# pr0g/ToyMeshPathTracer

Hardware: NVIDIA B200
Metric: Mrays/s (primary+bounce+shadow) (higher is better)
Workload: dtype f32

## Files before the change

toymeshpathtracer_b200/csrc/build_logic.cuh:

```cuda
#pragma once
#include "bvh.cuh"

namespace bld {

struct Box {
    float lox, loy, loz, hix, hiy, hiz;
};
TMPT_HD Box box_union(const Box& a, const Box& b) {
    return Box{fminf(a.lox, b.lox), fminf(a.loy, b.loy), fminf(a.loz, b.loz),
               fmaxf(a.hix, b.hix), fmaxf(a.hiy, b.hiy), fmaxf(a.hiz, b.hiz)};
}
TMPT_HD float box_half_area(const Box& b) {
    float dx = b.hix - b.lox, dy = b.hiy - b.loy, dz = b.hiz - b.loz;
    return dx * dy + dy * dz + dz * dx;
}

TMPT_HD uint32_t float_to_ordered(float f) {
    uint32_t u = ex::f2u(f);
    return (u & 0x80000000u) ? ~u : (u | 0x80000000u);
}
TMPT_HD float ordered_to_float(uint32_t u) {
    return ex::u2f((u & 0x80000000u) ? (u & 0x7FFFFFFFu) : ~u);
}

// ... 282 lines not shown
            const uint32_t wi = wideBase + (uint32_t)inner;
            refs[j] = wi;
            if (w.parent) w.parent[wi] = it.wide;
            outQueue[qBase + inner] = WorkItem{c[j], wi, it.depth + 1};
            ++inner;
        }
    }
    counter_max(&w.counters[3], (uint32_t)it.depth);
    float4* o = w.nodes + (size_t)it.wide * bvh::NODE_F4;
    o[0] = make_float4(lox[0], lox[1], lox[2], lox[3]);
    o[1] = make_float4(hix[0], hix[1], hix[2], hix[3]);
    o[2] = make_float4(loy[0], loy[1], loy[2], loy[3]);
    o[3] = make_float4(hiy[0], hiy[1], hiy[2], hiy[3]);
    o[4] = make_float4(loz[0], loz[1], loz[2], loz[3]);
    o[5] = make_float4(hiz[0], hiz[1], hiz[2], hiz[3]);
    o[6] = make_float4(ex::u2f(refs[0]), ex::u2f(refs[1]), ex::u2f(refs[2]), ex::u2f(refs[3]));
}

TMPT_HD void emit_single_leaf_root(const BinTree& t, const WideOut& w, int rootNode) {
    const int cnt = subtree_count(t, rootNode);
    const uint32_t first = counter_add(&w.counters[1], (uint32_t)cnt);
    counter_add(&w.counters[2], 1u);
    emit_leaf_tris(t, w, rootNode, first);
    const float4 lo = t.lo[rootNode], hi = t.hi[rootNode];
    const float F = 3.0e38f;
    float4* o = w.nodes;
    o[0] = make_float4(lo.x, F, F, F); o[1] = make_float4(hi.x, -F, -F, -F);
    o[2] = make_float4(lo.y, F, F, F); o[3] = make_float4(hi.y, -F, -F, -F);
    o[4] = make_float4(lo.z, F, F, F); o[5] = make_float4(hi.z, -F, -F, -F);
    o[6] = make_float4(ex::u2f(bvh::make_leaf_ref(first, cnt)), ex::u2f(bvh::NONE), ex::u2f(bvh::NONE), ex::u2f(bvh::NONE));
    accum_add(&w.sahAccum[1], box_half_area(Box{lo.x, lo.y, lo.z, hi.x, hi.y, hi.z}) * (float)cnt);
}


template <class LoadRow>
TMPT_HD void refit_wide_node(float4* nodes, float4* tris, const float* tris9, uint32_t node, float sceneMaxAbs, LoadRow ldnode) {
    float4* o = nodes + (size_t)node * bvh::NODE_F4;
    const float4 rf = o[6];
    const uint32_t refs[4] = {ex::f2u(rf.x), ex::f2u(rf.y), ex::f2u(rf.z), ex::f2u(rf.w)};
    float lo[3][4], hi[3][4];
    for (int k = 0; k < 4; ++k) {
        Box b{3.0e38f, 3.0e38f, 3.0e38f, -3.0e38f, -3.0e38f, -3.0e38f};
        if (refs[k] != bvh::NONE && bvh::ref_is_leaf(refs[k])) {
            const uint32_t first = bvh::leaf_first(refs[k]);
            for (int j = 0; j < bvh::leaf_count(refs[k]); ++j) {
                float4* slot = tris + (size_t)(first + j) * 3;
                const uint32_t id = ex::f2u(slot[0].w);
                const float* p = tris9 + (size_t)id * 9;
                const ex::V3 v0 = ex::v3(p[0], p[1], p[2]), v1 = ex::v3(p[3], p[4], p[5]), v2 = ex::v3(p[6], p[7], p[8]);
                const ex::V3 e1 = ex::sub(v1, v0), e2 = ex::sub(v2, v0);
                slot[0] = make_float4(v0.x, v0.y, v0.z, ex::u2f(id));
                slot[1] = make_float4(e1.x, e1.y, e1.z, 0.0f);
                slot[2] = make_float4(e2.x, e2.y, e2.z, 0.0f);
                Box tb = tri_box(p);
                const float dx = tb.hix - tb.lox, dy = tb.hiy - tb.loy, dz = tb.hiz - tb.loz;
                const float pad = pad_for(sqrtf(dx * dx + dy * dy + dz * dz), sceneMaxAbs);
                tb.lox -= pad; tb.loy -= pad; tb.loz -= pad; tb.hix += pad; tb.hiy += pad; tb.hiz += pad;
                b = box_union(b, tb);
            }
        } else if (refs[k] != bvh::NONE) {
            const float4 r0 = ldnode(refs[k], 0), r1 = ldnode(refs[k], 1), r2 = ldnode(refs[k], 2), r3 = ldnode(refs[k], 3), r4 = ldnode(refs[k], 4),
                         r5 = ldnode(refs[k], 5);
            b.lox = fminf(fminf(r0.x, r0.y), fminf(r0.z, r0.w)); b.hix = fmaxf(fmaxf(r1.x, r1.y), fmaxf(r1.z, r1.w));
            b.loy = fminf(fminf(r2.x, r2.y), fminf(r2.z, r2.w)); b.hiy = fmaxf(fmaxf(r3.x, r3.y), fmaxf(r3.z, r3.w));
            b.loz = fminf(fminf(r4.x, r4.y), fminf(r4.z, r4.w)); b.hiz = fmaxf(fmaxf(r5.x, r5.y), fmaxf(r5.z, r5.w));
        }
// ... 84 lines not shown
```

toymeshpathtracer_b200/csrc/bvh.cuh:

```cuda
#pragma once
#include "exact.cuh"
#include "sungrid.cuh"


#ifdef __CUDA_ARCH__
#define TMPT_LDG4(p) __ldg(p)
#else
#define TMPT_LDG4(p) (*(p))
#endif

namespace bvh {

constexpr uint32_t LEAF_BIT = 0x80000000u;
constexpr int MAX_LEAF_TRIS = 8;
constexpr int WIDTH = 4;
constexpr int NODE_F4 = 7;
constexpr int QNODE_ROWS = 4;
#ifndef TMPT_STACK_SIZE
#define TMPT_STACK_SIZE 128
#endif
constexpr int STACK_SIZE = TMPT_STACK_SIZE;
constexpr int MAX_TREE_DEPTH = (STACK_SIZE - 4) / 3;
constexpr uint32_t NONE = 0xFFFFFFFFu;
constexpr uint32_t STACK_OVERFLOW = 1;

TMPT_HD uint32_t make_leaf_ref(uint32_t firstSlot, int count) { return LEAF_BIT | (uint32_t(count - 1) << 28) | firstSlot; }
TMPT_HD bool ref_is_leaf(uint32_t r) { return (r & LEAF_BIT) != 0; }
TMPT_HD int leaf_count(uint32_t r) { return int((r >> 28) & 7u) + 1; }
TMPT_HD uint32_t leaf_first(uint32_t r) { return r & 0x0FFFFFFFu; }

struct SceneView {
    const float4* nodes;
    const float4* tris;
    const float* tris9;
    const float4* hitdata;
    uint32_t rootRef;
    int triCount;
    uint32_t* status;
    const uint4* qnodes;
    float farLimit;
    sun::View sun;
};

struct HitRec {
    int id;
    float t;
    float u, v;
};



TMPT_HD bool mt_exact(ex::V3 o, ex::V3 d, ex::V3 v0, ex::V3 e1, ex::V3 e2, float tMin, float tMax,
                      float& t, float& u, float& v) {
    const float Epsilon = 1e-5f;
    ex::V3 pvec = ex::cross(d, e2);
    float det = ex::dot(e1, pvec);
    float invDet = ex::rcp(det);
    ex::V3 tvec = ex::sub(o, v0);
    u = ex::mul(ex::dot(tvec, pvec), invDet);
    if ((det > -Epsilon && det < Epsilon) || u < 0.0f || u > 1.0f) return false;
    ex::V3 qvec = ex::cross(tvec, e1);
    v = ex::mul(ex::dot(d, qvec), invDet);
    if (v < 0.0f || ex::add(u, v) > 1.0f) return false;
    t = ex::mul(ex::dot(e2, qvec), invDet);
    return t >= tMin && t <= tMax;
}

TMPT_HD ex::V3 tri_normal(ex::V3 v0, ex::V3 v1, ex::V3 v2) { return ex::normalize(ex::cross(ex::sub(v1, v0), ex::sub(v2, v0))); }
TMPT_HD float4 ld_row_payload(const float4* p);
TMPT_HD void hit_payload(const SceneView& sc, int id, float u, float v, ex::V3& pos, ex::V3& normal) {
    ex::V3 v0, v1, v2;
    if (sc.hitdata) {
        const float4* h = sc.hitdata + (size_t)id * 3;
        const float4 a = ld_row_payload(h), b = ld_row_payload(h + 1), c = ld_row_payload(h + 2);
        v0 = ex::v3(a.x, a.y, a.z); v1 = ex::v3(b.x, b.y, b.z); v2 = ex::v3(c.x, c.y, c.z);
        normal = ex::v3(a.w, b.w, c.w);
    } else {
        const float* p = sc.tris9 + (size_t)id * 9;
        v0 = ex::v3(p[0], p[1], p[2]); v1 = ex::v3(p[3], p[4], p[5]); v2 = ex::v3(p[6], p[7], p[8]);
        normal = tri_normal(v0, v1, v2);
    }
    float w = ex::sub(ex::sub(1.0f, u), v);
    pos = ex::add(ex::add(ex::muls(v0, w), ex::muls(v1, u)), ex::muls(v2, v));
}

TMPT_HD float safe_dir(float d) { return fabsf(d) < 1.0e-20f ? copysignf(1.0e-20f, d) : d; }

struct TravStats {
    unsigned long long nodes = 0;
    unsigned long long tris = 0;
    unsigned long long iters = 0;
    unsigned long long culledPops = 0;
    unsigned long long leafWaits = 0;
    unsigned long long nodeWarps = 0;
    unsigned long long triWarps = 0;
    unsigned long long warpIters = 0;
    unsigned long long overflows = 0;
    unsigned long long depthOver[5] = {0, 0, 0, 0, 0};
    int maxSp = 0;
};

struct LocalStack {
    static constexpr bool kCanOverflow = false;
    unsigned long long e[STACK_SIZE];
    TMPT_HD bool put_if(bool push, int i, unsigned long long v) {
        if (push) e[i] = v;
        return push;
    }
    TMPT_HD unsigned long long get(int i) const { return *(const volatile unsigned long long*)&e[i]; }
    TMPT_HD bool overflowed() const { return false; }
    TMPT_HD void reset() {}
};
template <int S, int STRIDE>
struct SmemStack {
    static constexpr bool kCanOverflow = true;
    uint32_t col;
    bool ovf;
#ifdef __CUDA_ARCH__
    static __device__ __forceinline__ SmemStack make(const void* smemBase, uint32_t thread) {
        uint32_t a = (uint32_t)__cvta_generic_to_shared(smemBase) + thread * 8u, held;
        asm volatile("mov.u32 %0, %1;" : "=r"(held) : "r"(a));
        return SmemStack{held, false};
    }
    __device__ __forceinline__ bool put_if(bool push, int i, unsigned long long v) {
        const bool ok = push && i < S;
        if (ok) asm volatile("st.shared.u64 [%0], %1;" ::"r"(col + (uint32_t)i * (uint32_t)(STRIDE * 8)), "l"(v) : "memory");
        ovf = ovf || (push && !ok);
        return ok;
    }
    __device__ __forceinline__ unsigned long long get(int i) const {
        unsigned long long v;
// ... 313 lines not shown
#endif
    if (e == end) return false;
#ifdef __CUDA_ARCH__
    uint2 cur = __ldg(g.entries + e);
#else
    uint2 cur = g.entries[e];
#endif
    for (;;) {
        if (ex::u2f(cur.y) < w) return false;
        ++e;
        uint2 nxt = cur;
        if (e < end) {
#ifdef __CUDA_ARCH__
            nxt = __ldg(g.entries + e);
#else
            nxt = g.entries[e];
#endif
        }
        if (STATS) ++stats->tris;
        const uint32_t row0 = cur.x * 3u;
        const float4 a = ld_row_tri(sc.tris + row0), b = ld_row_tri(sc.tris + (row0 + 1u)), cc = ld_row_tri(sc.tris + (row0 + 2u));
        float t, bu, bv;
        if (mt_exact(p, l, ex::v3(a.x, a.y, a.z), ex::v3(b.x, b.y, b.z), ex::v3(cc.x, cc.y, cc.z), tMin, tMax, t, bu, bv)) return true;
        if (e >= end) return false;
        cur = nxt;
    }
}

struct WalkState {
    RayCtx r;
    ex::V3 o, d;
    HitRec best;
    uint32_t cur, triPos, triEnd;
    int sp;
    bool any;
};
TMPT_HD void walk_start(WalkState& w, const SceneView& sc, ex::V3 o, ex::V3 d, float tMax, bool any) {
    w.r = make_ray_ctx(o, d);
    w.o = o; w.d = d;
    w.best.id = -1; w.best.t = tMax; w.best.u = 0.0f; w.best.v = 0.0f;
    w.cur = ray_has_nan(o, d) ? NONE : sc.rootRef;
    w.triPos = 0; w.triEnd = 0;
    w.sp = 0;
    w.any = any;
}

TMPT_HD bool stats_any(bool pred) {
#ifdef __CUDA_ARCH__
    return __any_sync(__activemask(), pred);
#else
    return pred;
#endif
}
TMPT_HD bool stats_leader() {
#ifdef __CUDA_ARCH__
    const unsigned m = __activemask();
    unsigned lane;
    asm("mov.u32 %0, %%laneid;" : "=r"(lane));
    return (unsigned)(__ffs((int)m) - 1) == lane;
#else
    return true;
#endif
}

template <bool STATS, class Stack>
TMPT_HD bool walk_step(WalkState& w, const SceneView& sc, float tMin, float tMax, Stack& stack, TravStats* stats) {
    if (STATS) {
        ++stats->iters;
        const bool nodeAny = stats_any(w.cur != NONE && !ref_is_leaf(w.cur));
        if (stats_leader()) { ++stats->warpIters; stats->nodeWarps += nodeAny ? 1 : 0; }
    }
    if (w.cur != NONE && !ref_is_leaf(w.cur)) {
        if (STATS) ++stats->nodes;
        w.cur = node_step(sc, w.cur, w.r, tMin, w.best.t, stack, w.sp, w.any);
        if (STATS && w.sp > stats->maxSp) stats->maxSp = w.sp;
    }
    if (w.cur != NONE && ref_is_leaf(w.cur) && w.triPos == w.triEnd) {
        w.triPos = leaf_first(w.cur);
        w.triEnd = w.triPos + (uint32_t)leaf_count(w.cur);
        w.cur = NONE;
    }
    if (STATS) {
        if (w.cur != NONE && ref_is_leaf(w.cur)) ++stats->leafWaits;
        const bool triAny = stats_any(w.triPos < w.triEnd);
        if (stats_leader()) stats->triWarps += triAny ? 1 : 0;
    }
    const bool popping = w.cur == NONE && w.sp > 0;
    unsigned long long top = 0;
    if (popping) top = stack.get(w.sp - 1);
    if (w.triPos < w.triEnd) {
        if (STATS) ++stats->tris;
        if (tri_step(sc, w.triPos++, w.o, w.d, tMin, tMax, w.best) && w.any) return true;
    }
    if (popping) {
        --w.sp;
        if (ex::u2f((uint32_t)(top >> 32) & ~3u) <= w.best.t) w.cur = (uint32_t)top;
        else if (STATS) ++stats->culledPops;
    }
    const bool done = w.cur == NONE && w.triPos == w.triEnd && w.sp == 0;
    if (STATS && done) {
        const int lim[5] = {4, 8, 12, 16, 24};
        for (int k = 0; k < 5; ++k) stats->depthOver[k] += stats->maxSp > lim[k] ? 1 : 0;
        stats->maxSp = 0;
    }
    return done;
}

#ifdef __CUDA_ARCH__
// ... 12 lines not shown
            const int id = (int)ex::f2u(a.w);
            if (t < best.t || (t == best.t && best.id >= 0 && id < best.id)) { best.t = t; best.id = id; best.u = u; best.v = v; }
        }
    }
    return best;
}
TMPT_HD HitRec brute_force(const SceneView& sc, ex::V3 o, ex::V3 d, float tMin, float tMax) { return scan_all(sc.tris, sc.triCount, o, d, tMin, tMax); }

template <bool STATS>
TMPT_HD bool sun_query(const SceneView& sc, ex::V3 o, float tMin, float tMax, TravStats* stats) {
    const ex::V3 l = ex::v3(sc.sun.lx, sc.sun.ly, sc.sun.lz);
    if (ray_is_far(sc, o)) return scan_all(sc.tris, sc.triCount, o, l, tMin, tMax).id >= 0;
    return sun_occluded<STATS>(sc, o, l, tMin, tMax, stats);
}

template <bool ANY, bool STATS = false>
TMPT_HD HitRec traverse(const SceneView& sc, ex::V3 o, ex::V3 d, float tMin, float tMax, TravStats* stats = nullptr) {
    if (ray_is_far(sc, o)) return scan_all(sc.tris, sc.triCount, o, d, tMin, tMax);
    LocalStack stack;
    WalkState w;
    walk_start(w, sc, o, d, tMax, ANY);
    while (!walk_step<STATS>(w, sc, tMin, tMax, stack, stats)) {}
    return w.best;
}
template <bool ANY>
#ifdef __CUDA_ARCH__
__device__ __noinline__
#else
inline
#endif
HitRec traverse_again(const SceneView& sc, ex::V3 o, ex::V3 d, float tMin, float tMax) { return traverse<ANY, false>(sc, o, d, tMin, tMax); }

template <bool ANY, bool STATS, bool FAR, class Stack>
TMPT_HD HitRec traverse_with(Stack& stack, const SceneView& sc, ex::V3 o, ex::V3 d, float tMin, float tMax, TravStats* stats = nullptr) {
    if (FAR && ray_is_far(sc, o)) return scan_all(sc.tris, sc.triCount, o, d, tMin, tMax);
    WalkState w;
    walk_start(w, sc, o, d, tMax, ANY);
    while (!walk_step<STATS>(w, sc, tMin, tMax, stack, stats)) {}
    if (Stack::kCanOverflow && stack.overflowed()) {
        stack.reset();
        if (STATS) ++stats->overflows;
        if (!(ANY && w.best.id >= 0)) return traverse_again<ANY>(sc, o, d, tMin, tMax);
    }
    return w.best;
}

}
```

toymeshpathtracer_b200/csrc/integrator.cuh:

```cuda
#pragma once
#include "bvh.cuh"

namespace integ {

constexpr int kMaxDepth = 10;
constexpr float kMinT = 0.001f;
constexpr float kMaxT = 1.0e7f;

struct Camera {
    ex::V3 origin, lowerLeftCorner, horizontal, vertical, u, v, w;
    float lensRadius;
};

TMPT_HD void camera_get_ray(const Camera& c, float s, float t, uint32_t& rng, ex::V3& o, ex::V3& d) {
    float px, py;
    ex::random_in_unit_disk(rng, px, py);
    const float rdx = ex::mul(c.lensRadius, px), rdy = ex::mul(c.lensRadius, py);
    const ex::V3 offset = ex::add(ex::muls(c.u, rdx), ex::muls(c.v, rdy));
    o = ex::add(c.origin, offset);
    d = ex::normalize(ex::sub(ex::sub(ex::add(ex::add(c.lowerLeftCorner, ex::muls(c.horizontal, s)), ex::muls(c.vertical, t)), c.origin), offset));
}

TMPT_HD void primary_ray(const Camera& c, int x, int y, float invW, float invH, uint32_t& rng, ex::V3& o, ex::V3& d) {
    const float fv = ex::mul(ex::add((float)y, ex::random_float01(rng)), invH);
    const float fu = ex::mul(ex::add((float)x, ex::random_float01(rng)), invW);
    camera_get_ray(c, fu, fv, rng, o, d);
}

TMPT_HD ex::V3 sky(ex::V3 dir) {
    const float t = ex::mul(0.5f, ex::add(dir.y, 1.0f));
    const float a = ex::sub(1.0f, t);
    return ex::muls(ex::add(ex::v3(ex::mul(1.0f, a), ex::mul(1.0f, a), ex::mul(1.0f, a)), ex::muls(ex::v3(0.5f, 0.7f, 1.0f), t)), 0.5f);
}

TMPT_HD float sun_term(ex::V3 normal, ex::V3 rayDir, ex::V3 lightDir) {
    const ex::V3 nl = ex::dot(normal, rayDir) < 0.0f ? normal : ex::neg(normal);
    return fmaxf(0.0f, ex::dot(lightDir, nl));
}

// ... 2 lines not shown
    return ex::normalize(ex::sub(target, pos));
}

TMPT_HD ex::V3 unwind_step(float k, ex::V3 color) {
    const ex::V3 albedo = ex::v3(0.7f, 0.7f, 0.7f);
    const ex::V3 kLightColor = ex::v3(0.7f, 0.6f, 0.5f);
    const ex::V3 light = ex::add(ex::v3(0.0f, 0.0f, 0.0f), ex::muls(ex::mulv(albedo, kLightColor), k));
    return ex::add(light, ex::mulv(albedo, color));
}

TMPT_HD uchar4 resolve_pixel(ex::V3 sum, float sppRecip) {
    const ex::V3 c = ex::muls(sum, sppRecip);
    uchar4 px;
    px.x = ex::quantise(ex::sqrt_rn(c.x));
    px.y = ex::quantise(ex::sqrt_rn(c.y));
    px.z = ex::quantise(ex::sqrt_rn(c.z));
    px.w = 255;
    return px;
}

struct FirstHit {
    int id;
    float t;
    ex::V3 normal;
};

template <bool STATS = false, bool FAR = true, bool AOV = false, class Stack, class Scene>
TMPT_HD ex::V3 trace_path(Stack& stack, const Scene& sc, const Camera& cam, ex::V3 o, ex::V3 d, ex::V3 lightDir, uint32_t& rng,
                          unsigned long long& rays, bvh::TravStats* stats = nullptr, FirstHit* first = nullptr) {
    float kk[kMaxDepth];
    int depth = 0;
    ex::V3 color = ex::v3(0.0f, 0.0f, 0.0f);
    if (AOV) first->id = -1;
    while (depth < kMaxDepth) {
        ++rays;
        const bvh::HitRec h = bvh::traverse_with<false, STATS, FAR>(stack, sc, o, d, kMinT, kMaxT, stats);
        if (h.id < 0) { color = sky(d); break; }
        ex::V3 pos, normal;
        bvh::hit_payload(sc, h.id, h.u, h.v, pos, normal);
        if (AOV && depth == 0) { first->id = h.id; first->t = h.t; first->normal = normal; }
        ++rays;
#if defined(TMPT_SUN_ONLY) && TMPT_SUN_ONLY
        const bool shadowed = bvh::sun_occluded<STATS>(sc, pos, lightDir, kMinT, kMaxT, stats);
#else
        const bool shadowed = sc.sun.n > 0 ? bvh::sun_occluded<STATS>(sc, pos, lightDir, kMinT, kMaxT, stats)
                                           : bvh::traverse_with<true, STATS, FAR>(stack, sc, pos, lightDir, kMinT, kMaxT, stats).id >= 0;
#endif
        kk[depth] = shadowed ? 0.0f : sun_term(normal, d, lightDir);
        d = scatter_dir(pos, normal, rng);
        o = pos;
        ++depth;
    }
    for (int i = depth - 1; i >= 0; --i) color = unwind_step(kk[i], color);
    return color;
}

constexpr int kMaxChunkSamples = 8;
TMPT_HD int chunk_len(int spp) {
    const int c = spp / 32;
    return c < 1 ? 1 : c > kMaxChunkSamples ? kMaxChunkSamples : c;
}
TMPT_HD int chunk_count(int spp) { const int c = chunk_len(spp); return (spp + c - 1) / c; }

struct AovSums {
    ex::V3 normal;
    float t, hits;
    int id0;
};
TMPT_HD void aov_clear(AovSums& a) { a.normal = ex::v3(0.0f, 0.0f, 0.0f); a.t = 0.0f; a.hits = 0.0f; a.id0 = -1; }
TMPT_HD void aov_add_hit(AovSums& a, ex::V3 normal, float t) { a.normal = ex::add(a.normal, normal); a.t = ex::add(a.t, t); a.hits = ex::add(a.hits, 1.0f); }

TMPT_HD float4 radiance_of(ex::V3 sum, float sppRecip) {
    const ex::V3 c = ex::muls(sum, sppRecip);
    return make_float4(c.x, c.y, c.z, 1.0f);
}
TMPT_HD float4 normal_of(ex::V3 normalSum, float hits, float sppRecip) {
    const ex::V3 n = ex::muls(normalSum, sppRecip);
    return make_float4(n.x, n.y, n.z, ex::mul(hits, sppRecip));
}
// ... 58 lines not shown
```

toymeshpathtracer_b200/csrc/kernels.cu:

```cuda
#include <cooperative_groups.h>
#include <cuda_runtime.h>

#include <atomic>
#include <chrono>
#include <cmath>
#include <cstdarg>
#include <cstdio>
#include <cstdlib>
#include <cstring>
#include <mutex>
#include <new>
#include <string>
#include <vector>

#include "build_logic.cuh"
#include "common.h"
#include "denoise.cuh"
#include "integrator.cuh"
#ifndef TMPT_EXPERIMENTS
#define TMPT_EXPERIMENTS 0
#endif

namespace tmpt {
static thread_local std::string g_err;
// ... 15 lines not shown
extern "C" int tmpt_device_count(void) {
    int n = 0;
    if (cudaGetDeviceCount(&n) != cudaSuccess) { cudaGetLastError(); return 0; }
    return n;
}

#define CU_TRY(expr)                                                                                       \
    do {                                                                                                   \
        cudaError_t e_ = (expr);                                                                           \
        if (e_ != cudaSuccess) return tmpt::fail(e_ == cudaErrorMemoryAllocation ? TMPT_ERR_OOM : TMPT_ERR_CUDA, \
                                                 "%s:%d %s: %s", __FILE__, __LINE__, #expr, cudaGetErrorString(e_)); \
    } while (0)
#define LAUNCH(kernel, grid, block, smem, stream, ...)      \
    do {                                                    \
        kernel<<<(grid), (block), (smem), (stream)>>>(__VA_ARGS__); \
        tmpt::count_launch();                               \
    } while (0)

static inline int div_up(long long a, long long b) { return (int)((a + b - 1) / b); }

struct tmpt_scene {
    int device = 0;
    int triCount = 0;
    int smCount = 148;
    cudaStream_t stream = nullptr;
    float* d_tris9 = nullptr;
    float4* d_nodes = nullptr;
    uint4* d_qnodes = nullptr;
    float4* d_tris = nullptr;
    float4* d_hitdata = nullptr;
    uint32_t* d_parent = nullptr;
    uint32_t* d_pending = nullptr;
    uint32_t* d_bounds = nullptr;
    uint32_t* d_status = nullptr;
    uint32_t* d_tileCounter = nullptr;
    unsigned long long* d_rayCount = nullptr;
    unsigned long long* d_fetchCounter = nullptr;
    uint8_t* d_frame = nullptr;
    size_t frameBytes = 0;
    float4* d_accum = nullptr;
    size_t accumBytes = 0;
    float4* d_sum = nullptr;
    size_t sumBytes = 0;
    void* d_outs[4] = {};
    size_t outsBytes[4] = {};
    int progW = 0, progH = 0, progChunks = -1;
    int progAdaptive = -1;
    uint32_t* d_adN = nullptr;
    float2* d_adStat = nullptr;
    uint32_t *d_adFlags = nullptr, *d_adOffs = nullptr, *d_adTotals = nullptr;
    uint2* d_adList = nullptr;
    unsigned int* d_adActive = nullptr;
    size_t adPixels = 0;
    int32_t* d_samples = nullptr;
    size_t samplesBytes = 0;
    float4* d_denoise = nullptr;
    size_t denoiseBytes = 0;
    char* d_stage = nullptr;
    char* h_stage = nullptr;
    size_t stageBytes = 0;
    std::mutex hostCallMutex;
    uint32_t *d_sunStart = nullptr, *d_sunCount = nullptr;
    uint2* d_sunEntries = nullptr;
    uint32_t sunEntriesCap = 0, sunEntries = 0;
    uint64_t sunBytes = 0;
    size_t sunStartCap = 0, sunCountCap = 0;
// ... 341 lines not shown
        const bld::WorkItem* inQ = (level & 1) ? qB : qA;
        bld::WorkItem* outQ = (level & 1) ? qA : qB;
        for (uint32_t i = tid; i < cnt; i += nthreads) {
            const bld::WorkItem it{__ldcg(&inQ[i].bnode), __ldcg(&inQ[i].wide), __ldcg(&inQ[i].depth)};
            bld::collapse_node(t, w, it, outQ, &counts[(level + 1) % 3]);
        }
        grid.sync();
    }
}
struct LoadNodeRowCg {
    const float4* nodes;
    __device__ float4 operator()(uint32_t n, int row) const { return __ldcg(nodes + (size_t)n * bvh::NODE_F4 + row); }
};
__global__ void k_refit_pending(const float4* __restrict__ nodes, uint32_t count, uint32_t* __restrict__ pending) {
    const uint32_t i = blockIdx.x * blockDim.x + threadIdx.x;
    if (i < count) pending[i] = (uint32_t)bld::wide_inner_children(nodes, i);
}
__global__ void k_refit_wide(float4* nodes, float4* tris, const float* __restrict__ tris9, const uint32_t* __restrict__ parent, uint32_t* pending,
                             uint32_t count, const uint32_t* __restrict__ bounds) {
    const uint32_t i = blockIdx.x * blockDim.x + threadIdx.x;
    if (i >= count || bld::wide_inner_children(nodes, i) != 0) return;
    const bld::Box scene = load_scene_box(bounds);
    const float maxAbs = fmaxf(fmaxf(fmaxf(fabsf(scene.lox), fabsf(scene.hix)), fmaxf(fabsf(scene.loy), fabsf(scene.hiy))),
                               fmaxf(fabsf(scene.loz), fabsf(scene.hiz)));
    uint32_t node = i;
    for (;;) {
        bld::refit_wide_node(nodes, tris, tris9, node, maxAbs, LoadNodeRowCg{nodes});
        if (node == 0) break;
        __threadfence();
        const uint32_t p = parent[node];
        if (atomicSub(&pending[p], 1u) != 1u) break;
        node = p;
    }
}
__global__ void k_quantize_nodes(const float4* __restrict__ nodesF, uint4* __restrict__ qnodes, uint32_t count) {
    const uint32_t i = blockIdx.x * blockDim.x + threadIdx.x;
    if (i < count) bld::quantize_node(nodesF, qnodes, i);
}
__global__ void k_collapse_root_leaf(bld::BinTree t, bld::WideOut w, int rootNode) { bld::emit_single_leaf_root(t, w, rootNode); }

__device__ __forceinline__ void flush_stats(unsigned long long* stats, unsigned long long rays, const bvh::TravStats& ts, unsigned long long hits) {
    unsigned long long v[16] = {rays, ts.nodes, ts.tris, hits, ts.iters, ts.culledPops, ts.leafWaits, ts.nodeWarps, ts.triWarps, ts.warpIters,
                                ts.overflows, ts.depthOver[0], ts.depthOver[1], ts.depthOver[2], ts.depthOver[3], ts.depthOver[4]};
    for (int k = 0; k < 16; ++k) {
        for (int o = 16; o > 0; o >>= 1) v[k] += __shfl_xor_sync(0xffffffffu, v[k], o);
        if ((threadIdx.x & 31) == 0 && v[k]) atomicAdd(&stats[k], v[k]);
    }
}

template <int MODE, bool STATS>
__global__ void __launch_bounds__(128) k_hit_scene(bvh::SceneView sc, const float* __restrict__ rays6, long long nRays, float tMin, float tMax,
                                                    int* __restrict__ outID, float* __restrict__ outT, float* __restrict__ outPos,
                                                    float* __restrict__ outNormal, unsigned long long* __restrict__ stats) {
    bvh::TravStats ts;
    unsigned long long nr = 0, nh = 0;
    for (long long i = (long long)blockIdx.x * blockDim.x + threadIdx.x; i < nRays; i += (long long)gridDim.x * blockDim.x) {
        const float* r = rays6 + i * 6;
        const ex::V3 o = ex::v3(r[0], r[1], r[2]), d = ex::v3(r[3], r[4], r[5]);
        bvh::HitRec h;
        if (MODE == TMPT_HIT_BRUTE) h = bvh::brute_force(sc, o, d, tMin, tMax);
        else if (MODE == TMPT_HIT_SUN) {
            h.id = sc.sun.n > 0 && bvh::sun_query<STATS>(sc, o, tMin, tMax, &ts) ? 1 : -1;
            h.t = 0.0f; h.u = 0.0f; h.v = 0.0f;
        } else if (MODE == TMPT_HIT_ANY) h = bvh::traverse<true, STATS>(sc, o, d, tMin, tMax, &ts);
        else h = bvh::traverse<false, STATS>(sc, o, d, tMin, tMax, &ts);
        if (STATS) { ++nr; nh += h.id >= 0; }
// ... 275 lines not shown
                    depth = 0; newRay = true; newAny = false;
                }
            }
            if (newRay) {
                ++rays;
                bvh::walk_start(w, p.sc, no, ndir, integ::kMaxT, newAny);
                state = ST_WALK;
            }
            if (__all_sync(FULL, state == ST_IDLE)) break;
        }
        if (state == ST_WALK) {
            if (bvh::walk_step<STATS>(w, p.sc, integ::kMinT, integ::kMaxT, stack, &ts))
                state = w.any ? ST_SHADOW_DONE : w.best.id < 0 ? ST_PATH_END : ST_HIT;
        }
    }
    if (STATS) flush_stats(p.stats, rays, ts, 0);
    for (int o = 16; o > 0; o >>= 1) rays += __shfl_xor_sync(FULL, rays, o);
    if (lane == 0 && rays) atomicAdd(p.rayCount, rays);
}

#endif

template <int THREADS, int MINB, int GATE, bool AOV = false, bool LIST = false>
__global__ void __launch_bounds__(THREADS, MINB) k_render_paths(const RenderParams p) {
    constexpr unsigned FULL = 0xffffffffu;
    const int lane = threadIdx.x & 31;
    bvh::LocalStack stack;
    float kk[integ::kMaxDepth];
    unsigned long long rays = 0;
    bool havePath = false, done = false, exhausted = false;
    uint32_t rng = 0, pix = 0, loc = 0, cl = 0;
    bool hasItem = false;
    int depth = 0;
    ex::V3 sum = ex::v3(0.0f, 0.0f, 0.0f), o = sum, d = sum, nsum = sum;
    float tsum = 0.0f;
    const float invW = ex::divf(1.0f, (float)p.width), invH = ex::divf(1.0f, (float)p.height);
    const unsigned long long totalItems = (unsigned long long)p.numTiles * (unsigned long long)p.chunks * 32ull;
    for (;;) {
        const unsigned need = __ballot_sync(FULL, !havePath && !done);
        const unsigned tracing = __ballot_sync(FULL, havePath);
        if (need && (__popc(need) >= GATE || tracing == 0)) {
            bool wantItem = !havePath && !done && (cl & 0xFFu) == 0u;
            if (wantItem && hasItem) {
                const int xl = (int)(loc & 0xFFFFu), rb = (int)(loc >> 16);
                if (LIST) {
                    __stcs(&p.accum[(size_t)(cl >> 8) * p.listLen + loc], make_float4(sum.x, sum.y, sum.z, 0.0f));
                } else if (p.useAccum) {
                    const size_t a = ((size_t)(AOV ? (cl >> 8) & 0xFFFFu : cl >> 8) * p.bandRows + rb) * p.localWidth + xl;
                    __stcs(&p.accum[a], make_float4(sum.x, sum.y, sum.z, AOV ? (float)(cl >> 24) : 0.0f));
                    if (AOV) __stcs(&p.accum[a + (size_t)p.chunks * p.bandRows * p.localWidth], make_float4(nsum.x, nsum.y, nsum.z, tsum));
                } else {
                    const uchar4 px = integ::resolve_pixel(sum, ex::divf(1.0f, (float)p.spp));
                    if (p.frame) p.frame[(size_t)(pix >> 16) * p.width + (pix & 0xFFFFu)] = px;
                    else p.outStripes[(size_t)(p.bandRow0 + rb) * p.localWidth + xl] = px;
                }
                hasItem = false;
            }
            while (__any_sync(FULL, wantItem)) {
                const unsigned want = __ballot_sync(FULL, wantItem);
                if (exhausted) { if (wantItem) { done = true; wantItem = false; } break; }
                const int cnt = __popc(want);
                unsigned long long base = 0;
                if (lane == __ffs((int)want) - 1) base = atomicAdd(p.laneCounter, (unsigned long long)cnt);
                base = __shfl_sync(FULL, base, __ffs((int)want) - 1);
                exhausted = base + (unsigned long long)cnt >= totalItems;
                if (wantItem) {
// ... 11 lines not shown
                                                     (uint32_t)p.width * (uint32_t)p.height);
                                pix = en.x;
                                loc = e;
                                cl = ((uint32_t)chunk << 8) | (uint32_t)integ::kMaxChunkSamples;
                                sum = ex::v3(0.0f, 0.0f, 0.0f);
                                hasItem = true;
                                wantItem = false;
                            }
                            continue;
                        }
                        const int tx = (int)(tile % (uint32_t)p.tilesX), ty = (int)(tile / (uint32_t)p.tilesX);
                        const int xl = tx * 8 + (int)(li & 7u), rb = ty * 4 + (int)(li >> 3);
                        const int r = p.bandRow0 + rb;
                        int x, y;
                        if (xl < p.localWidth && r < p.ownedRows && local_to_global(xl, r, p.stripeRows, p.rank, p.world, p.width, x, y)) {
                            const int gchunk = p.chunk0 + chunk;
                            rng = ex::chunk_seed((uint32_t)gchunk, (uint32_t)y * (uint32_t)p.width + (uint32_t)x, (uint32_t)p.width * (uint32_t)p.height);
                            const int s0 = gchunk * p.chunkLen;
                            const int left = (s0 + p.chunkLen < p.spp ? s0 + p.chunkLen : p.spp) - s0;
                            pix = (uint32_t)x | ((uint32_t)y << 16);
                            loc = (uint32_t)xl | ((uint32_t)rb << 16);
                            cl = ((uint32_t)chunk << 8) | (uint32_t)left;
                            sum = ex::v3(0.0f, 0.0f, 0.0f);
                            if (AOV) { nsum = sum; tsum = 0.0f; }
                            hasItem = true;
                            wantItem = false;
                        }
                    }
                }
            }
            if (!havePath && !done && (cl & 0xFFu) != 0u) {
                integ::primary_ray(p.cam, (int)(pix & 0xFFFFu), (int)(pix >> 16), invW, invH, rng, o, d);
                depth = 0;
                havePath = true;
            }
        }
        if (__all_sync(FULL, done)) break;
        bool hit = false;
        bvh::HitRec h;
        h.id = -1;
        if (havePath) {
            ++rays;
            h = bvh::traverse_with<false, false, false>(stack, p.sc, o, d, integ::kMinT, integ::kMaxT);
            hit = h.id >= 0;
        }
        ex::V3 pos = ex::v3(0.0f, 0.0f, 0.0f), normal = pos;
        bool shadowed = false;
        if (hit) {
            bvh::hit_payload(p.sc, h.id, h.u, h.v, pos, normal);
            ++rays;
            shadowed = p.sc.sun.n > 0 ? bvh::sun_occluded<false>(p.sc, pos, p.lightDir, integ::kMinT, integ::kMaxT, nullptr)
                                      : bvh::traverse_with<true, false, false>(stack, p.sc, pos, p.lightDir, integ::kMinT, integ::kMaxT).id >= 0;
        }
        if (havePath) {
            bool ended = false;
            ex::V3 color = ex::v3(0.0f, 0.0f, 0.0f);
            if (AOV && depth == 0) {
                if (p.triangle && p.chunk0 == 0 && cl == (uint32_t)min(p.chunkLen, p.spp))
                    p.triangle[(size_t)(pix >> 16) * p.width + (pix & 0xFFFFu)] = h.id;
                if (hit) { nsum = ex::add(nsum, normal); tsum = ex::add(tsum, h.t); cl += 1u << 24; }
            }
            if (hit) {
                kk[depth] = shadowed ? 0.0f : integ::sun_term(normal, d, p.lightDir);
                d = integ::scatter_dir(pos, normal, rng);
                o = pos;
                ++depth;
                ended = depth == integ::kMaxDepth;
            } else {
                color = integ::sky(d);
                ended = true;
            }
            if (ended) {
                for (int i = depth - 1; i >= 0; --i) color = integ::unwind_step(kk[i], color);
                sum = ex::add(sum, color);
                --cl;
                havePath = false;
            }
        }
    }
    for (int k = 16; k > 0; k >>= 1) rays += __shfl_xor_sync(FULL, rays, k);
    if (lane == 0 && rays) atomicAdd(p.rayCount, rays);
}

constexpr long long kSunBigCells = 2048;
__device__ __forceinline__ void sun_bin_cell(const sun::View& g, const sun::Tri2& t, int slot, int cx, int cy, bool fill, uint32_t* cellCount,
// ... 278 lines not shown
struct DevBuf {
    T* p = nullptr;
    ~DevBuf() { if (p) cudaFree(p); }
    cudaError_t alloc(size_t n) { return cudaMalloc((void**)&p, (n ? n : 1) * sizeof(T)); }
};

constexpr int kTreeTooDeep = -100;

int build_bvh(tmpt_scene* s, unsigned flags) {
    const int n = s->triCount;
    cudaStream_t st = s->stream;
    const float cInner = getenv("TMPT_SAH_CI") ? (float)atof(getenv("TMPT_SAH_CI")) : 1.0f, cTri = 1.0f;
    int coopAttr = 0;
    CU_TRY(cudaDeviceGetAttribute(&coopAttr, cudaDevAttrCooperativeLaunch, s->device));
    const bool coop = coopAttr != 0 && !(getenv("TMPT_BUILD_HOSTLOOP") && atoi(getenv("TMPT_BUILD_HOSTLOOP")) != 0);
    const int maxLeaf = getenv("TMPT_SAH_MAXLEAF") ? std::max(1, std::min(bvh::MAX_LEAF_TRIS, atoi(getenv("TMPT_SAH_MAXLEAF")))) : bvh::MAX_LEAF_TRIS;

    struct Arr { void* p = nullptr; };
    Arr bounds, primA, primB, visits, counters, qCount, keysA, keysB, left, right, parent, first, lo, hi, sah, qA, qB, pLo, pHi, primFinal, nodeCounter, tqA, tqB;
    DevBuf<char> arena;
    {
        const size_t N = (size_t)n;
        struct Req { Arr* a; size_t bytes; };
        const Req reqs[] = {{&bounds, 6 * 4}, {&primA, N * 4}, {&primB, N * 4}, {&visits, N * 4}, {&counters, 4 * 4}, {&qCount, 4 * 4}, {&keysA, N * 8},
                            {&keysB, N * 8}, {&left, 2 * N * 4}, {&right, 2 * N * 4}, {&parent, 2 * N * 4}, {&first, 2 * N * 4}, {&lo, 2 * N * 16},
                            {&hi, 2 * N * 16}, {&sah, 2 * 4}, {&qA, N * sizeof(bld::WorkItem)}, {&qB, N * sizeof(bld::WorkItem)}, {&pLo, N * 16},
                            {&pHi, N * 16}, {&primFinal, N * 4}, {&nodeCounter, 4}, {&tqA, N * sizeof(SahTask)}, {&tqB, N * sizeof(SahTask)}};
        size_t total = 0;
        for (const Req& r : reqs) total += (r.bytes + 255) & ~(size_t)255;
        CU_TRY(arena.alloc(total));
        size_t off = 0;
        for (const Req& r : reqs) { r.a->p = arena.p + off; off += (r.bytes + 255) & ~(size_t)255; }
    }
    CU_TRY(cudaMalloc((void**)&s->d_nodes, (size_t)n * (bvh::NODE_F4 + 3 + 3) * sizeof(float4) + ((size_t)n * 2 + 8) * sizeof(uint32_t)));
    s->d_tris = s->d_nodes + (size_t)n * bvh::NODE_F4;
    s->d_hitdata = s->d_tris + (size_t)n * 3;
    s->d_parent = (uint32_t*)(s->d_hitdata + (size_t)n * 3);
    s->d_pending = s->d_parent + n;
    s->d_bounds = s->d_pending + n;
    CU_TRY(cudaMemsetAsync(s->d_parent, 0, sizeof(uint32_t), st));

    uint32_t* const d_bounds = (uint32_t*)bounds.p; uint32_t* const d_primA = (uint32_t*)primA.p; uint32_t* const d_primB = (uint32_t*)primB.p;
    uint32_t* const d_visits = (uint32_t*)visits.p; uint32_t* const d_counters = (uint32_t*)counters.p; uint32_t* const d_qCount = (uint32_t*)qCount.p;
    uint64_t* const d_keysA = (uint64_t*)keysA.p; uint64_t* const d_keysB = (uint64_t*)keysB.p;
    int* const d_left = (int*)left.p; int* const d_right = (int*)right.p; int* const d_parent = (int*)parent.p; int* const d_first = (int*)first.p;
    float4* const d_lo = (float4*)lo.p; float4* const d_hi = (float4*)hi.p; float* const d_sah = (float*)sah.p;
    bld::WorkItem* const d_qA = (bld::WorkItem*)qA.p; bld::WorkItem* const d_qB = (bld::WorkItem*)qB.p;
    const uint32_t initBounds[6] = {0xFFFFFFFFu, 0xFFFFFFFFu, 0xFFFFFFFFu, 0u, 0u, 0u};
    CU_TRY(cudaMemcpyAsync(d_bounds, initBounds, sizeof initBounds, cudaMemcpyHostToDevice, st));
    CU_TRY(cudaMemsetAsync(d_visits, 0, (size_t)n * sizeof(uint32_t), st));
    CU_TRY(cudaMemsetAsync(d_counters, 0, 4 * sizeof(uint32_t), st));
    CU_TRY(cudaMemsetAsync(d_sah, 0, 2 * sizeof(float), st));
    CU_TRY(cudaMemsetAsync(d_parent, 0xFF, 2 * (size_t)n * sizeof(int), st));

    const int B = 256, G = div_up(n, B);
    LAUNCH(k_prim_bounds, G, B, 0, st, s->d_tris9, n, d_bounds);
    LAUNCH(k_hitdata, G, B, 0, st, s->d_tris9, n, s->d_hitdata);
    bld::BinTree t{n, d_keysA, d_left, d_right, d_parent, d_lo, d_hi, d_first, d_visits};
    bld::SahParams sp{cInner, cTri, maxLeaf};
    const uint32_t* primOrder = d_primA;
    int rootIsLeaf = (n == 1);
    if (flags & TMPT_BUILD_LBVH) {
        LAUNCH(k_morton, G, B, 0, st, s->d_tris9, n, d_bounds, d_keysA, d_primA);
        const int passes = 16;
        const int sortSmem = 16 * SORT_THREADS * (int)sizeof(uint32_t);
        CU_TRY(cudaFuncSetAttribute(k_radix_sort, cudaFuncAttributeMaxDynamicSharedMemorySize, sortSmem));
        LAUNCH(k_radix_sort, 1, SORT_THREADS, sortSmem, st, d_keysA, d_primA, d_keysB, d_primB, n, passes);
        LAUNCH(k_leaf_boxes, G, B, 0, st, s->d_tris9, d_primA, n, d_bounds, cTri, d_lo, d_hi, d_first);
        if (n > 1) {
            LAUNCH(k_karras, div_up(n - 1, B), B, 0, st, t);
            LAUNCH(k_refit, G, B, 0, st, t, sp);
        }
// ... 99 lines not shown
            }
        }
    }
    uint32_t hc[4]; float hs[2]; uint32_t hb[6];
    CU_TRY(cudaMemcpyAsync(hc, d_counters, sizeof hc, cudaMemcpyDeviceToHost, st));
    CU_TRY(cudaMemcpyAsync(hs, d_sah, sizeof hs, cudaMemcpyDeviceToHost, st));
    CU_TRY(cudaMemcpyAsync(hb, d_bounds, sizeof hb, cudaMemcpyDeviceToHost, st));
    CU_TRY(cudaStreamSynchronize(st));
    CU_TRY(cudaGetLastError());
    s->info.node_count = (int)hc[0];
    s->info.leaf_count = (int)hc[2];
    s->info.max_depth = (int)hc[3] + 1;
    s->info.max_leaf_tris = bvh::MAX_LEAF_TRIS;
    for (int k = 0; k < 3; ++k) {
        s->info.bounds_min[k] = bld::ordered_to_float(hb[k]);
        s->info.bounds_max[k] = bld::ordered_to_float(hb[3 + k]);
    }
    {
        const float dx = s->info.bounds_max[0] - s->info.bounds_min[0], dy = s->info.bounds_max[1] - s->info.bounds_min[1],
                    dz = s->info.bounds_max[2] - s->info.bounds_min[2];
        const float rootArea = dx * dy + dy * dz + dz * dx;
        s->info.sah_cost = rootArea > 0.0f ? (cInner * hs[0] + cTri * hs[1]) / rootArea : 0.0f;
    }
    if ((int)hc[1] != n) return tmpt::fail(TMPT_ERR_CUDA, "BVH build lost triangles: %u slots for %d triangles", hc[1], n);
#if TMPT_QNODES
    CU_TRY(cudaMalloc((void**)&s->d_qnodes, ((size_t)hc[0] * bvh::QNODE_STRIDE) * sizeof(uint4)));
    LAUNCH(k_quantize_nodes, div_up((int)hc[0], 128), 128, 0, st, s->d_nodes, s->d_qnodes, hc[0]);
#endif
    if (3 * s->info.max_depth + 4 > bvh::STACK_SIZE) {
        tmpt::fail(TMPT_ERR_ARG, "BVH is %d levels deep; the traversal stack (%d entries) supports %d", s->info.max_depth, bvh::STACK_SIZE,
                   (bvh::STACK_SIZE - 4) / 3);
        return kTreeTooDeep;
    }
    s->info.device_bytes = (uint64_t)n * 9 * 4 + (uint64_t)hc[0] * (bvh::NODE_F4 + (TMPT_QNODES ? bvh::QNODE_STRIDE : 0)) * 16 + (uint64_t)n * 48 + (uint64_t)n * 48;
    s->view.nodes = s->d_nodes;
    s->view.qnodes = s->d_qnodes;
    s->view.tris = s->d_tris;
    s->view.tris9 = s->d_tris9;
    s->view.hitdata = s->d_hitdata;
    s->view.rootRef = 0u;
    s->view.triCount = n;
    s->view.status = s->d_status;
    s->view.farLimit = bvh_far_limit(s->info);
    return TMPT_OK;
}

constexpr unsigned long long kSunMaxEntries = 256ull << 20;
static ex::V3 host_light_dir() { return ex::normalize(ex::v3(-0.7f, 1.0f, 0.5f)); }
static int build_sun_grid(tmpt_scene* s, int n, cudaStream_t st) {
    static const int forced = getenv("TMPT_SUN_GRID") ? atoi(getenv("TMPT_SUN_GRID")) : -1;
    s->view.sun = sun::View{};
    s->info.device_bytes -= s->sunBytes;
    s->sunBytes = 0; s->sunEntries = 0;
    if (forced == 0 || n <= 0) return TMPT_OK;
    static const bool trace = getenv("TMPT_SUN_TRACE") != nullptr;
    auto now = [] { return std::chrono::duration<double, std::milli>(std::chrono::steady_clock::now().time_since_epoch()).count(); };
    const double t0 = now();
    sun::View g;
    if (!sun::setup_view(s->info.bounds_min, s->info.bounds_max, host_light_dir(), g)) return TMPT_OK;
    const double t1 = now();
    int cells = forced > 0 ? std::min(std::max(forced, 1), 8192) : sun::default_cells_per_side(n);
    for (;; cells /= 2) {
        if (cells < (forced > 0 ? 1 : 32)) return TMPT_OK;
        sun::set_resolution(g, cells);
        const long long nCells = (long long)cells * cells;
        const int nBlocks = (int)((nCells + kScanBlock - 1) / kScanBlock);
        const size_t needStart = (size_t)nCells + 1, needCount = (size_t)nCells + nBlocks + 2 + n;
        if (s->sunStartCap < needStart) {
            cudaFree(s->d_sunStart); s->d_sunStart = nullptr; s->sunStartCap = 0;
            CU_TRY(cudaMalloc((void**)&s->d_sunStart, needStart * sizeof(uint32_t)));
            s->sunStartCap = needStart;
        }
// ... 102 lines not shown
        } else {
            s->view = bvh::SceneView{nullptr, nullptr, nullptr, nullptr, bvh::NONE, 0, s->d_status, nullptr, 0.0f};
        }
        CU_TRY(cudaEventRecord(s->ev1, s->stream));
        CU_TRY(cudaStreamSynchronize(s->stream));
        float ms = 0.0f;
        CU_TRY(cudaEventElapsedTime(&ms, s->ev0, s->ev1));
        s->info.build_ms = ms;
        return TMPT_OK;
    };
    rc = body();
    if (rc != TMPT_OK) { tmpt_scene_destroy(s); return rc; }
    *outScene = s;
    return TMPT_OK;
}

extern "C" int tmpt_scene_refit(tmpt_scene* s, const float* tris9, int triCount, double* seconds) {
    if (!s || (triCount > 0 && !tris9)) return tmpt::fail(TMPT_ERR_ARG, "tmpt_scene_refit: NULL scene / triangles");
    if (triCount != s->triCount) return tmpt::fail(TMPT_ERR_ARG, "tmpt_scene_refit: %d triangles, the scene was built with %d", triCount, s->triCount);
    if (seconds) *seconds = 0.0;
    if (triCount == 0) return TMPT_OK;
    DeviceGuard guard(s->device);
    if (!guard.ok) return tmpt::fail(TMPT_ERR_CUDA, "tmpt_scene_refit: cudaSetDevice(%d) failed", s->device);
    cudaStream_t st = s->stream;
    const int n = triCount, B = 256, G = div_up(n, B), nodes = s->info.node_count;
    CU_TRY(cudaEventRecord(s->ev0, st));
    CU_TRY(cudaMemcpyAsync(s->d_tris9, tris9, (size_t)n * 9 * sizeof(float), cudaMemcpyHostToDevice, st));
    const uint32_t initBounds[6] = {0xFFFFFFFFu, 0xFFFFFFFFu, 0xFFFFFFFFu, 0u, 0u, 0u};
    CU_TRY(cudaMemcpyAsync(s->d_bounds, initBounds, sizeof initBounds, cudaMemcpyHostToDevice, st));
    LAUNCH(k_prim_bounds, G, B, 0, st, s->d_tris9, n, s->d_bounds);
    LAUNCH(k_hitdata, G, B, 0, st, s->d_tris9, n, s->d_hitdata);
    LAUNCH(k_refit_pending, div_up(nodes, 128), 128, 0, st, s->d_nodes, (uint32_t)nodes, s->d_pending);
    LAUNCH(k_refit_wide, div_up(nodes, 128), 128, 0, st, s->d_nodes, s->d_tris, s->d_tris9, s->d_parent, s->d_pending, (uint32_t)nodes, s->d_bounds);
#if TMPT_QNODES
    LAUNCH(k_quantize_nodes, div_up(nodes, 128), 128, 0, st, s->d_nodes, s->d_qnodes, (uint32_t)nodes);
#endif
    uint32_t hb[6];
    CU_TRY(cudaMemcpyAsync(hb, s->d_bounds, sizeof hb, cudaMemcpyDeviceToHost, st));
    CU_TRY(cudaStreamSynchronize(st));
    CU_TRY(cudaGetLastError());
    for (int k = 0; k < 3; ++k) {
        s->info.bounds_min[k] = bld::ordered_to_float(hb[k]);
        s->info.bounds_max[k] = bld::ordered_to_float(hb[3 + k]);
    }
    {
        const int grc = build_sun_grid(s, n, st);
        if (grc != TMPT_OK) return grc;
    }
    CU_TRY(cudaEventRecord(s->ev1, st));
    CU_TRY(cudaStreamSynchronize(st));
    CU_TRY(cudaGetLastError());
    s->view.farLimit = bvh_far_limit(s->info);
    s->probeW = 0;
    float ms = 0.0f;
    CU_TRY(cudaEventElapsedTime(&ms, s->ev0, s->ev1));
    if (seconds) *seconds = ms * 1e-3;
    return TMPT_OK;
}

extern "C" void tmpt_scene_destroy(tmpt_scene* s) {
    if (!s) return;
    DeviceGuard guard(s->device);
    if (s->stream) cudaStreamSynchronize(s->stream);
    cudaFree(s->d_tris9); cudaFree(s->d_nodes); cudaFree(s->d_qnodes); cudaFree(s->d_status);
    cudaFree(s->d_tileCounter); cudaFree(s->d_rayCount); cudaFree(s->d_fetchCounter); cudaFree(s->d_frame); cudaFree(s->d_accum); cudaFree(s->d_sum);
    for (void* o : s->d_outs) cudaFree(o);
// ... 874 lines not shown
```

Baseline: 7786.

## Skip self-leaf intersection for rays leaving axis-aligned planar leaves

At build and refit time, each triangle is marked with its leaf ref when every triangle in that leaf lies in the same axis-aligned plane as it does. When a hit point lies exactly on that plane, the bounce and shadow rays from it skip that leaf during traversal, because with tMin > 0 they cannot hit a coplanar triangle. This avoids redundant triangle tests on the surface the ray just left. The cost is an extra per-triangle array, an extra build kernel, and a compare plus a global load in hit_payload on every hit.

```diff
diff --git a/toymeshpathtracer_b200/csrc/build_logic.cuh b/toymeshpathtracer_b200/csrc/build_logic.cuh
--- a/toymeshpathtracer_b200/csrc/build_logic.cuh
+++ b/toymeshpathtracer_b200/csrc/build_logic.cuh
@@ -338,6 +338,31 @@
     accum_add(&w.sahAccum[1], box_half_area(Box{lo.x, lo.y, lo.z, hi.x, hi.y, hi.z}) * (float)cnt);
 }
 
+
+TMPT_HD uint32_t axis_planes(const float* p) {
+    return (p[0] == p[3] && p[0] == p[6] ? 1u : 0u) | (p[1] == p[4] && p[1] == p[7] ? 2u : 0u) | (p[2] == p[5] && p[2] == p[8] ? 4u : 0u);
+}
+TMPT_HD void mark_plane_leaves(const float4* nodes, const float4* tris, const float* tris9, uint32_t node, uint32_t* planeLeaf) {
+    const float4 rf = nodes[(size_t)node * bvh::NODE_F4 + 6];
+    const uint32_t refs[4] = {ex::f2u(rf.x), ex::f2u(rf.y), ex::f2u(rf.z), ex::f2u(rf.w)};
+    for (int k = 0; k < 4; ++k) {
+        if (refs[k] == bvh::NONE || !bvh::ref_is_leaf(refs[k])) continue;
+        const uint32_t first = bvh::leaf_first(refs[k]);
+        const int cnt = bvh::leaf_count(refs[k]);
+        const float* p0 = tris9 + (size_t)ex::f2u(tris[(size_t)first * 3].w) * 9;
+        uint32_t leafMask = 7u;
+        for (int j = 0; j < cnt; ++j) {
+            const float* p = tris9 + (size_t)ex::f2u(tris[(size_t)(first + j) * 3].w) * 9;
+            for (int a = 0; a < 3; ++a)
+                if (!(p[a] == p0[a] && p[3 + a] == p0[a] && p[6 + a] == p0[a])) leafMask &= ~(1u << a);
+        }
+        for (int j = 0; j < cnt; ++j) {
+            const uint32_t id = ex::f2u(tris[(size_t)(first + j) * 3].w);
+            const uint32_t own = axis_planes(tris9 + (size_t)id * 9);
+            planeLeaf[id] = own != 0u && own == leafMask ? refs[k] : bvh::NONE;
+        }
+    }
+}
 
 template <class LoadRow>
 TMPT_HD void refit_wide_node(float4* nodes, float4* tris, const float* tris9, uint32_t node, float sceneMaxAbs, LoadRow ldnode) {
diff --git a/toymeshpathtracer_b200/csrc/bvh.cuh b/toymeshpathtracer_b200/csrc/bvh.cuh
--- a/toymeshpathtracer_b200/csrc/bvh.cuh
+++ b/toymeshpathtracer_b200/csrc/bvh.cuh
@@ -40,6 +40,7 @@
     const uint4* qnodes;
     float farLimit;
     sun::View sun;
+    const uint32_t* planeLeaf;
 };
 
 struct HitRec {
@@ -68,7 +69,8 @@
 
 TMPT_HD ex::V3 tri_normal(ex::V3 v0, ex::V3 v1, ex::V3 v2) { return ex::normalize(ex::cross(ex::sub(v1, v0), ex::sub(v2, v0))); }
 TMPT_HD float4 ld_row_payload(const float4* p);
-TMPT_HD void hit_payload(const SceneView& sc, int id, float u, float v, ex::V3& pos, ex::V3& normal) {
+TMPT_HD uint32_t origin_skip_ref(const uint32_t* planeLeaf, int id, ex::V3 v0, ex::V3 v1, ex::V3 v2, ex::V3 pos);
+TMPT_HD void hit_payload(const SceneView& sc, int id, float u, float v, ex::V3& pos, ex::V3& normal, uint32_t* skipRef = nullptr) {
     ex::V3 v0, v1, v2;
     if (sc.hitdata) {
         const float4* h = sc.hitdata + (size_t)id * 3;
@@ -82,6 +84,14 @@
     }
     float w = ex::sub(ex::sub(1.0f, u), v);
     pos = ex::add(ex::add(ex::muls(v0, w), ex::muls(v1, u)), ex::muls(v2, v));
+    if (skipRef) *skipRef = origin_skip_ref(sc.planeLeaf, id, v0, v1, v2, pos);
+}
+
+TMPT_HD uint32_t origin_skip_ref(const uint32_t* planeLeaf, int id, ex::V3 v0, ex::V3 v1, ex::V3 v2, ex::V3 pos) {
+    const bool onX = v0.x == v1.x && v0.x == v2.x && pos.x == v0.x;
+    const bool onY = v0.y == v1.y && v0.y == v2.y && pos.y == v0.y;
+    const bool onZ = v0.z == v1.z && v0.z == v2.z && pos.z == v0.z;
+    return (onX || onY || onZ) && planeLeaf ? planeLeaf[id] : 0xFFFFFFFFu;
 }
 
 TMPT_HD float safe_dir(float d) { return fabsf(d) < 1.0e-20f ? copysignf(1.0e-20f, d) : d; }
@@ -97,6 +107,8 @@
     unsigned long long warpIters = 0;
     unsigned long long overflows = 0;
     unsigned long long depthOver[5] = {0, 0, 0, 0, 0};
+    unsigned long long skippedTris = 0;
+    unsigned long long skippedLeaves = 0;
     int maxSp = 0;
 };
 
@@ -476,15 +488,17 @@
     ex::V3 o, d;
     HitRec best;
     uint32_t cur, triPos, triEnd;
+    uint32_t skipRef;
     int sp;
     bool any;
 };
-TMPT_HD void walk_start(WalkState& w, const SceneView& sc, ex::V3 o, ex::V3 d, float tMax, bool any) {
+TMPT_HD void walk_start(WalkState& w, const SceneView& sc, ex::V3 o, ex::V3 d, float tMax, bool any, uint32_t skipRef = NONE) {
     w.r = make_ray_ctx(o, d);
     w.o = o; w.d = d;
     w.best.id = -1; w.best.t = tMax; w.best.u = 0.0f; w.best.v = 0.0f;
     w.cur = ray_has_nan(o, d) ? NONE : sc.rootRef;
     w.triPos = 0; w.triEnd = 0;
+    w.skipRef = skipRef;
     w.sp = 0;
     w.any = any;
 }
@@ -518,6 +532,10 @@
         if (STATS) ++stats->nodes;
         w.cur = node_step(sc, w.cur, w.r, tMin, w.best.t, stack, w.sp, w.any);
         if (STATS && w.sp > stats->maxSp) stats->maxSp = w.sp;
+    }
+    if (w.cur == w.skipRef) {
+        if (STATS && w.cur != NONE) { ++stats->skippedLeaves; stats->skippedTris += (unsigned long long)leaf_count(w.cur); }
+        w.cur = NONE;
     }
     if (w.cur != NONE && ref_is_leaf(w.cur) && w.triPos == w.triEnd) {
         w.triPos = leaf_first(w.cur);
@@ -596,10 +614,11 @@
 HitRec traverse_again(const SceneView& sc, ex::V3 o, ex::V3 d, float tMin, float tMax) { return traverse<ANY, false>(sc, o, d, tMin, tMax); }
 
 template <bool ANY, bool STATS, bool FAR, class Stack>
-TMPT_HD HitRec traverse_with(Stack& stack, const SceneView& sc, ex::V3 o, ex::V3 d, float tMin, float tMax, TravStats* stats = nullptr) {
+TMPT_HD HitRec traverse_with(Stack& stack, const SceneView& sc, ex::V3 o, ex::V3 d, float tMin, float tMax, TravStats* stats = nullptr,
+                             uint32_t skipRef = NONE) {
     if (FAR && ray_is_far(sc, o)) return scan_all(sc.tris, sc.triCount, o, d, tMin, tMax);
     WalkState w;
-    walk_start(w, sc, o, d, tMax, ANY);
+    walk_start(w, sc, o, d, tMax, ANY, skipRef);
     while (!walk_step<STATS>(w, sc, tMin, tMax, stack, stats)) {}
     if (Stack::kCanOverflow && stack.overflowed()) {
         stack.reset();
diff --git a/toymeshpathtracer_b200/csrc/integrator.cuh b/toymeshpathtracer_b200/csrc/integrator.cuh
--- a/toymeshpathtracer_b200/csrc/integrator.cuh
+++ b/toymeshpathtracer_b200/csrc/integrator.cuh
@@ -5,6 +5,7 @@
 
 constexpr int kMaxDepth = 10;
 constexpr float kMinT = 0.001f;
+static_assert(kMinT > 0.0f, "bvh::origin_skip_ref is exact only for tMin > 0");
 constexpr float kMaxT = 1.0e7f;
 
 struct Camera {
@@ -73,19 +74,20 @@
     int depth = 0;
     ex::V3 color = ex::v3(0.0f, 0.0f, 0.0f);
     if (AOV) first->id = -1;
+    uint32_t skipRef = bvh::NONE;
     while (depth < kMaxDepth) {
         ++rays;
-        const bvh::HitRec h = bvh::traverse_with<false, STATS, FAR>(stack, sc, o, d, kMinT, kMaxT, stats);
+        const bvh::HitRec h = bvh::traverse_with<false, STATS, FAR>(stack, sc, o, d, kMinT, kMaxT, stats, skipRef);
         if (h.id < 0) { color = sky(d); break; }
         ex::V3 pos, normal;
-        bvh::hit_payload(sc, h.id, h.u, h.v, pos, normal);
+        bvh::hit_payload(sc, h.id, h.u, h.v, pos, normal, &skipRef);
         if (AOV && depth == 0) { first->id = h.id; first->t = h.t; first->normal = normal; }
         ++rays;
 #if defined(TMPT_SUN_ONLY) && TMPT_SUN_ONLY
         const bool shadowed = bvh::sun_occluded<STATS>(sc, pos, lightDir, kMinT, kMaxT, stats);
 #else
         const bool shadowed = sc.sun.n > 0 ? bvh::sun_occluded<STATS>(sc, pos, lightDir, kMinT, kMaxT, stats)
-                                           : bvh::traverse_with<true, STATS, FAR>(stack, sc, pos, lightDir, kMinT, kMaxT, stats).id >= 0;
+                                           : bvh::traverse_with<true, STATS, FAR>(stack, sc, pos, lightDir, kMinT, kMaxT, stats, skipRef).id >= 0;
 #endif
         kk[depth] = shadowed ? 0.0f : sun_term(normal, d, lightDir);
         d = scatter_dir(pos, normal, rng);
diff --git a/toymeshpathtracer_b200/csrc/kernels.cu b/toymeshpathtracer_b200/csrc/kernels.cu
--- a/toymeshpathtracer_b200/csrc/kernels.cu
+++ b/toymeshpathtracer_b200/csrc/kernels.cu
@@ -71,6 +71,7 @@
     uint32_t* d_parent = nullptr;
     uint32_t* d_pending = nullptr;
     uint32_t* d_bounds = nullptr;
+    uint32_t* d_planeLeaf = nullptr;
     uint32_t* d_status = nullptr;
     uint32_t* d_tileCounter = nullptr;
     unsigned long long* d_rayCount = nullptr;
@@ -478,6 +479,11 @@
         if (atomicSub(&pending[p], 1u) != 1u) break;
         node = p;
     }
+}
+__global__ void k_plane_leaves(const float4* __restrict__ nodes, const float4* __restrict__ tris, const float* __restrict__ tris9, uint32_t count,
+                               uint32_t* __restrict__ planeLeaf) {
+    const uint32_t i = blockIdx.x * blockDim.x + threadIdx.x;
+    if (i < count) bld::mark_plane_leaves(nodes, tris, tris9, i, planeLeaf);
 }
 __global__ void k_quantize_nodes(const float4* __restrict__ nodesF, uint4* __restrict__ qnodes, uint32_t count) {
     const uint32_t i = blockIdx.x * blockDim.x + threadIdx.x;
@@ -819,6 +825,7 @@
     uint32_t rng = 0, pix = 0, loc = 0, cl = 0;
     bool hasItem = false;
     int depth = 0;
+    uint32_t skipRef = bvh::NONE;
     ex::V3 sum = ex::v3(0.0f, 0.0f, 0.0f), o = sum, d = sum, nsum = sum;
     float tsum = 0.0f;
     const float invW = ex::divf(1.0f, (float)p.width), invH = ex::divf(1.0f, (float)p.height);
@@ -896,6 +903,7 @@
             if (!havePath && !done && (cl & 0xFFu) != 0u) {
                 integ::primary_ray(p.cam, (int)(pix & 0xFFFFu), (int)(pix >> 16), invW, invH, rng, o, d);
                 depth = 0;
+                skipRef = bvh::NONE;
                 havePath = true;
             }
         }
@@ -905,16 +913,17 @@
         h.id = -1;
         if (havePath) {
             ++rays;
-            h = bvh::traverse_with<false, false, false>(stack, p.sc, o, d, integ::kMinT, integ::kMaxT);
+            h = bvh::traverse_with<false, false, false>(stack, p.sc, o, d, integ::kMinT, integ::kMaxT, nullptr, skipRef);
             hit = h.id >= 0;
         }
         ex::V3 pos = ex::v3(0.0f, 0.0f, 0.0f), normal = pos;
         bool shadowed = false;
         if (hit) {
-            bvh::hit_payload(p.sc, h.id, h.u, h.v, pos, normal);
+            bvh::hit_payload(p.sc, h.id, h.u, h.v, pos, normal, &skipRef);
             ++rays;
             shadowed = p.sc.sun.n > 0 ? bvh::sun_occluded<false>(p.sc, pos, p.lightDir, integ::kMinT, integ::kMaxT, nullptr)
-                                      : bvh::traverse_with<true, false, false>(stack, p.sc, pos, p.lightDir, integ::kMinT, integ::kMaxT).id >= 0;
+                                      : bvh::traverse_with<true, false, false>(stack, p.sc, pos, p.lightDir, integ::kMinT, integ::kMaxT, nullptr,
+                                                                               skipRef).id >= 0;
         }
         if (havePath) {
             bool ended = false;
@@ -1259,12 +1268,13 @@
         size_t off = 0;
         for (const Req& r : reqs) { r.a->p = arena.p + off; off += (r.bytes + 255) & ~(size_t)255; }
     }
-    CU_TRY(cudaMalloc((void**)&s->d_nodes, (size_t)n * (bvh::NODE_F4 + 3 + 3) * sizeof(float4) + ((size_t)n * 2 + 8) * sizeof(uint32_t)));
+    CU_TRY(cudaMalloc((void**)&s->d_nodes, (size_t)n * (bvh::NODE_F4 + 3 + 3) * sizeof(float4) + ((size_t)n * 3 + 8) * sizeof(uint32_t)));
     s->d_tris = s->d_nodes + (size_t)n * bvh::NODE_F4;
     s->d_hitdata = s->d_tris + (size_t)n * 3;
     s->d_parent = (uint32_t*)(s->d_hitdata + (size_t)n * 3);
     s->d_pending = s->d_parent + n;
     s->d_bounds = s->d_pending + n;
+    s->d_planeLeaf = s->d_bounds + 8;
     CU_TRY(cudaMemsetAsync(s->d_parent, 0, sizeof(uint32_t), st));
 
     uint32_t* const d_bounds = (uint32_t*)bounds.p; uint32_t* const d_primA = (uint32_t*)primA.p; uint32_t* const d_primB = (uint32_t*)primB.p;
@@ -1430,12 +1440,15 @@
                    (bvh::STACK_SIZE - 4) / 3);
         return kTreeTooDeep;
     }
-    s->info.device_bytes = (uint64_t)n * 9 * 4 + (uint64_t)hc[0] * (bvh::NODE_F4 + (TMPT_QNODES ? bvh::QNODE_STRIDE : 0)) * 16 + (uint64_t)n * 48 + (uint64_t)n * 48;
+    LAUNCH(k_plane_leaves, div_up((int)hc[0], 128), 128, 0, st, s->d_nodes, s->d_tris, s->d_tris9, hc[0], s->d_planeLeaf);
+    s->info.device_bytes = (uint64_t)n * 9 * 4 + (uint64_t)hc[0] * (bvh::NODE_F4 + (TMPT_QNODES ? bvh::QNODE_STRIDE : 0)) * 16 + (uint64_t)n * 48 + (uint64_t)n * 48 +
+                           (uint64_t)n * 4;
     s->view.nodes = s->d_nodes;
     s->view.qnodes = s->d_qnodes;
     s->view.tris = s->d_tris;
     s->view.tris9 = s->d_tris9;
     s->view.hitdata = s->d_hitdata;
+    s->view.planeLeaf = s->d_planeLeaf;
     s->view.rootRef = 0u;
     s->view.triCount = n;
     s->view.status = s->d_status;
@@ -1604,6 +1617,7 @@
     LAUNCH(k_hitdata, G, B, 0, st, s->d_tris9, n, s->d_hitdata);
     LAUNCH(k_refit_pending, div_up(nodes, 128), 128, 0, st, s->d_nodes, (uint32_t)nodes, s->d_pending);
     LAUNCH(k_refit_wide, div_up(nodes, 128), 128, 0, st, s->d_nodes, s->d_tris, s->d_tris9, s->d_parent, s->d_pending, (uint32_t)nodes, s->d_bounds);
+    LAUNCH(k_plane_leaves, div_up(nodes, 128), 128, 0, st, s->d_nodes, s->d_tris, s->d_tris9, (uint32_t)nodes, s->d_planeLeaf);
 #if TMPT_QNODES
     LAUNCH(k_quantize_nodes, div_up(nodes, 128), 128, 0, st, s->d_nodes, s->d_qnodes, (uint32_t)nodes);
 #endif
```

After: 7798, median of 6. No clear change (+0.1%).
